# compbioproj-cdna-to-genome-map-align/gmap-2024

Hardware: AMD Instinct MI355X
Metric: aligned cDNA reads/sec (2 kb, GRCh38) at 1/2/4/8 MI355X; DP HBM GB/s vs peak (higher is better)
Workload: dtype int32

## Files before the change

### gmap-2024_amd/csrc/s2c_kernel.hip

```cpp
#include <cstdlib>

#include "dp_device.h"
#include <climits>

namespace gmapdp {

constexpr int kS2K = 8;
constexpr int kS2EqualNotSplicing = 9;
constexpr int kS2EnoughConsec = 32;
constexpr int kS2GreedyConsec = 100;
constexpr int kS2ExonDefn = 30;
constexpr int kS2MinTerminal = 8;
constexpr int kS2MaxNactive = 100;
constexpr int kS2MaxSkipped = 3;
constexpr int kS2ScoreRestrict = 10;
constexpr int kS2TenThousand = 8192;
constexpr int kS2FinalTolerance = 20;
constexpr int kS2MaxNalignments = 10;
constexpr int kS2Sufflookback = 60, kS2Nsufflookback = 5;
constexpr int kS2ExtraBounds = 20;
constexpr int kS2cCap = 4096;

#ifdef GMAPDP_OI_TIMING
__device__ unsigned long long g_s2_marks[2][16];
__device__ unsigned int g_s2_wave[3][16384];
__device__ unsigned long long g_s2_sub[2][8];
#define S2_SUB_DECL() unsigned long long _sub_t0 = 0
#define S2_SUB_T0() (_sub_t0 = wall_clock64())
#define S2_SUB(k) (W.sub[k] += wall_clock64() - _sub_t0, W.subn[k]++)
#define S2_MARK(k)                                                  \
  do {                                                              \
    if (threadIdx.x == 0) {                                         \
      atomicAdd(&g_s2_marks[0][k], (unsigned long long)wall_clock64()); \
      atomicAdd(&g_s2_marks[1][k], 1ull);                           \
    }                                                               \
  } while (0)
#define S2_COUNT(k, v)                                             \
  do {                                                              \
    if (threadIdx.x == 0) atomicAdd(&g_s2_marks[0][k], (unsigned long long)(v)); \
  } while (0)
#else
#define S2_MARK(k) \
  do {             \
  } while (0)
#define S2_COUNT(k, v) \
  do {                 \
  } while (0)
#define S2_SUB_DECL() (void)0
#define S2_SUB_T0() (void)0
#define S2_SUB(k) (void)0
#endif

constexpr int kS2NoPositions = 0, kS2Coverage = 1, kS2Chained = 2, kS2Overflow = -2, kS2Domain = -3;

struct __attribute__((aligned(16))) S2Hit {
  int consec, root, tracei, pred;
};
struct S2Diag {
  uint32_t diagonal;
  int querystart, queryend, nconsecutive, dominatedp, pad_;
  double score;
};
struct S2Path {
  int cell;
  int n;
  uint32_t start, end;
};
struct S2Scratch {
  size_t diff, run, off, minact, maxact, first, proc, diags, ord, tmp, hits, maps, sc, cand, keep, paths, pq, ph, lh,
      sbuf, total;
  int sortn;
};
__host__ __device__ inline int s2_pow2(int n) {
  int p = 64;
  while (p < n) p <<= 1;
  return p;
}
__host__ __device__ inline S2Scratch s2_scratch(int ql, int T, int nd) {
  S2Scratch s;
  const size_t Q = (size_t)ql + 1, D = (size_t)(nd > 0 ? nd : 1), H = (size_t)(T > 0 ? T : 1);
  s.diff = 0;
  s.run = align16(s.diff + 4 * Q);
  s.off = align16(s.run + 8 * Q);
  s.minact = align16(s.off + 4 * Q);
  s.maxact = align16(s.minact + 4 * Q);
  s.first = align16(s.maxact + 4 * Q);
  s.proc = align16(s.first + 4 * Q);
  s.diags = align16(s.proc + 4 * Q);
  s.ord = align16(s.diags + sizeof(S2Diag) * D);
  s.tmp = align16(s.ord + 4 * D);
  s.hits = align16(s.tmp + 4 * D);
  s.maps = align16(s.hits + sizeof(S2Hit) * H);
  s.sc = align16(s.maps + 4 * H);
  s.cand = align16(s.sc + 4 * H);
  s.keep = align16(s.cand + 4 * H);
  s.paths = align16(s.keep + 4 * H);
  s.pq = align16(s.paths + sizeof(S2Path) * H);
  s.ph = align16(s.pq + 4 * Q);
  s.lh = align16(s.ph + 4 * Q);
  s.sortn = s2_pow2((int)(H > D ? H : D));
  s.sbuf = align16(s.lh + 8 * Q);
  s.total = align16(s.sbuf + 4 * (size_t)s.sortn);
  return s;
}

__device__ __forceinline__ int wave_incl_sum(int x, int lane) {
#pragma unroll
  for (int off = 1; off < 64; off <<= 1) {
    const int y = __shfl_up(x, off, 64);
    if (lane >= off) x += y;
  }
  return x;
}
__device__ __forceinline__ int wave_incl_max(int x, int lane) {
#pragma unroll
  for (int off = 1; off < 64; off <<= 1) {
    const int y = __shfl_up(x, off, 64);
    if (lane >= off) x = max(x, y);
  }
  return x;
}
__device__ __forceinline__ int wave_max_i(int x) {
#pragma unroll
  for (int off = 32; off >= 1; off >>= 1) x = max(x, __shfl_xor(x, off, 64));
  return x;
}
__device__ __forceinline__ int wave_sum_i(int x) {
#pragma unroll
  for (int off = 32; off >= 1; off >>= 1) x += __shfl_xor(x, off, 64);
  return x;
}
__device__ __forceinline__ void wave_sync() { __syncthreads(); }

template <class Less>
__device__ void wave_sort(int lane, int n, const int* in, int* out, int* sbuf, Less less) {
  if (n <= 0) return;
  const int NN = s2_pow2(n);
  for (int i = lane; i < NN; i += 64) sbuf[i] = i < n ? i : -1;
  wave_sync();
  auto lt = [&](int x, int y) {
    if (x < 0) return false;
    if (y < 0) return true;
    const int vx = in[x], vy = in[y];
    if (less(vx, vy)) return true;
    if (less(vy, vx)) return false;
    return x < y;
  };
  for (int size = 2; size <= NN; size <<= 1) {
    for (int stride = size >> 1; stride > 0; stride >>= 1) {
      for (int i = lane; i < NN; i += 64) {
        const int j = i ^ stride;
        if (j > i) {
          const int a = sbuf[i], b = sbuf[j];
          const bool up = (i & size) == 0;
          if (up ? lt(b, a) : lt(a, b)) {
            sbuf[i] = b;
            sbuf[j] = a;
          }
        }
      }
      wave_sync();
    }
  }
  for (int i = lane; i < n; i += 64) out[i] = in[sbuf[i]];
  wave_sync();
}

template <class F>
__device__ __forceinline__ void fill_range(int lane, uint32_t* dst, int a, int b, F f) {
  for (int q = a + lane; q <= b; q += 64) dst[q] = f(q);
}

struct S2Best {
  int consec, root, pp, ph, score, tracei;
// ... 543 lines not shown
  }
  s2_uniform(b);
  bool donep = false;
  int last_tr = -1;
  if (np > 0 && b.consec < kS2EnoughConsec) {
    S2_SUB_T0();
    S2Pref pf;
    pf.load(W, np);
    const uint64_t dm = ballot(W.lane < np && W.lane > nlookback && (q - pf.q) - kS2K > lookback);
    const int kmax = dm ? __ffsll((long long)dm) - 1 : (np <= 64 ? np - 1 : 64);
    int fdummy = 0, lt = -1, from = 0;
    S2_SUB(1);
    int st;
    S2_SUB_T0();
    st = s2_dloop_fast(W, pf, np, kmax, q, position, b, W.splicingp != 0, false, fdummy, lt);
    S2_SUB(2);
    S2_SUB_T0();
    if (st == 2) from = 64;
    if (!st) {
      const int kg = kmax >= 64 ? 63 : kmax;
      S2Pref pg = pf;
      for (;;) {
        int nb = from;
        st = s2_dloop_multi(W, pg, np, kg, q, position, b, W.splicingp != 0, false, fdummy, lt, from, &nb);
        if (st != 2) break;
        from = nb;
        pg.load(W, np, from);
      }
      if (st == 1 && kmax >= 64 && b.consec < kS2EnoughConsec) {
        st = 2;
        from = 64;
      }
    }
    S2_SUB(3);
    S2_SUB_T0();
    if (st == 1) np = 0;
    if (st != 1) last_tr = lt;
    S2EntryCache ec;
    for (int kk = from; kk < np && b.consec < kS2EnoughConsec && !donep; kk++) {
      const int eq = kk < kS2Pref ? __builtin_amdgcn_readlane(pf.q, kk) : ec.get(W, np, kk).q;
      if (kk > nlookback && (q - eq) - kS2K > lookback) donep = true;
      int qd;
      (void)s2_entry_eval(W, pf, ec, np, kk, 0, q, position, last_tr, b, W.splicingp != 0, &qd);
    }
    S2_SUB(4);
  }
  s2_uniform(b);
  if (b.pp < 0) {
    b.tracei = ++W.tracectr;
    b.score = kS2K;
  }
  return b;
}

__device__ __forceinline__ void s2_store_link(S2W& W, int offq, int hit, const S2Best& b) {
  if (W.lane == 0) {
    W.hits[offq + hit] = S2Hit{b.consec, b.root, b.tracei, b.ph};
    W.sc[offq + hit] = b.score;
  }
}

__device__ __forceinline__ void s2_mult(S2W& W, int q, int offq, int low, int high, int np, const S2E& last) {
  int* fr = s2_fr;
  const int nhits = high - low;
  if (np == 0) {
    for (int i = W.lane; i < nhits; i += 64) {
      W.hits[offq + low + i] = S2Hit{kS2K, (int)W.maps[offq + low + i], W.tracectr + 1 + i, -1};
      W.sc[offq + low + i] = kS2K;
    }
    W.tracectr += nhits;
    wave_sync();
    return;
  }
  const int adq = q - last.q;
  int maxadj = 0, maxnon = 0, nfr = 0;
  S2EntryCache ec;
  for (int n = 0; n < np && n < 128; n++) {
    const S2E e = ec.get(W, np, n);
    const int qd = q - e.q;
    if (n > kS2Nsufflookback && n > 1 && qd - kS2K > kS2Sufflookback) break;
    if (n <= 1 || qd - kS2K <= kS2Sufflookback / 2) maxadj = n;
    if (n <= kS2Nsufflookback || qd - kS2K <= kS2Sufflookback) maxnon = n;
    if (W.lane == 0) fr[n] = e.n > 0 ? 0 : -1;
    nfr = n + 1;
  }
  wave_sync();
  int overall = 0, adjf = last.n > 0 ? 0 : -1;
  for (int i = 0; i < nhits; i++) {
    const uint32_t position = W.maps[offq + low + i];
    S2HV u;
    if (s2_adj(W, last, adjf, adq, position, u) && u.consec + adq > overall) overall = u.consec + adq;
  }
  adjf = last.n > 0 ? 0 : -1;
  for (int i = 0; i < nhits; i++) {
    const uint32_t position = W.maps[offq + low + i];
    S2Best b;
    int maxseen;
    S2HV u;
    if (s2_adj(W, last, adjf, adq, position, u)) {
      b = {u.consec + adq, u.root, last.q, u.hit, u.score + adq, u.tracei};
      maxseen = maxadj;
    } else {
      b = {kS2K, (int)position, -1, -1, 0, -1};
      maxseen = maxnon;
    }
    if (overall < kS2GreedyConsec) {
      int last_tr = -1;
      for (int kk = 0; kk < np && b.consec < kS2EnoughConsec && kk <= maxseen && kk < nfr; kk++) {
        const int f = s2_u(s2_fr[kk]);
        if (f != -1) {
          const S2E e = ec.get(W, np, kk);
          const int nf = s2_eval(W, e, f, q, position, last_tr, b, true);
          wave_sync();
          if (W.lane == 0) fr[kk] = nf;
          wave_sync();
        }
      }
    }
    if (b.pp < 0) {
      b.tracei = ++W.tracectr;
      b.score = kS2K;
    }
    s2_store_link(W, offq, low + i, b);
  }
  wave_sync();
}

struct S2Run {
  int score, consec, tracei, root, hit, q, pushed, np;
};
__device__ __forceinline__ void s2_run_write(S2Hit* hits, int* sc, int* alist, int lane, int off, int hit,
                                             int prev, uint32_t map, int qq, S2Run L, uint64_t Mm) {
  if (!((Mm >> lane) & 1ull)) return;
  const uint64_t below = Mm & ((1ull << lane) - 1ull);
  const int r = __popcll(below);
  const int dq = qq - L.q;
  hits[off + hit] = S2Hit{L.consec + dq, L.root, L.tracei, below ? prev : L.hit};
  sc[off + hit] = L.score + dq;
  alist[off] = hit;
  const int sl = (L.pushed + r) & (kS2Ring - 1);
  s2_ring.map[sl] = map;
  s2_ring.score[sl] = L.score + dq;
  s2_ring.consec[sl] = L.consec + dq;
  s2_ring.tracei[sl] = L.tracei;
  s2_ring.root[sl] = L.root;
  s2_ring.hit[sl] = off + hit;
  const int ms = (L.np + r) & (kS2Meta - 1);
  s2_ring.eq[ms] = qq;
  s2_ring.en[ms] = 1;
  s2_ring.eoff[ms] = off;
  s2_ring.estart[ms] = L.pushed + r;
}

__device__ __forceinline__ void s2_sweep(S2W& W, const int32_t* npq, int nq, const int* lowa, const int* higha,
                                         const uint32_t* rmapa, int qstart, int qend) {
  const int lane = W.lane;
  auto npos = [&](int q) { return q < nq ? npq[q] : 0; };
  int q = 0, np = 0;
  for (int i = lane; i < qstart; i += 64) W.actn[i] = 0;
  q = qstart;
  while (q <= qend && npos(q) <= 0) {
    if (lane == 0) W.actn[q] = 0;
    q++;
  }
  if (q <= qend) {
    const int n = npos(q), offq = W.off[q];
    for (int i = lane; i < n; i += 64) {
      W.hits[offq + i] = S2Hit{kS2K, 0, -1, -1};
      W.sc[offq + i] = kS2K;
    }
  }
  wave_sync();
  int grand_score = 0, grand_q = -1, grand_hit = -1, nskipped = 0, min_hits = 1000000, specific_q = -1,
      specific_low = 0, specific_high = 0;
  uint32_t grand_map = 0;
  S2E last = {0, 0, 0, 0, false};
  int cb = -1, m_n = 0, m_off = 0, m_low = 0, m_high = 0;
  uint32_t m_rmap = 0;
#ifdef GMAPDP_OI_TIMING
  unsigned long long t_one = 0, t_mult = 0, t_tail = 0, t_meta = 0, t0c = 0;
#define S2_T0() t0c = wall_clock64()
#define S2_TACC(acc) (acc += wall_clock64() - t0c, t0c = wall_clock64())
#else
#define S2_T0() (void)0
#define S2_TACC(acc) (void)0
#endif
  while (q <= qend) {
    S2_T0();
    W.tracectr = s2_u(W.tracectr);
    W.pushed = s2_u(W.pushed);
    if ((q & ~63) != cb) {
      cb = q & ~63;
      const int qq = cb + lane;
      const bool in = qq <= qend;
      m_n = qq < nq ? npq[qq] : 0;
      m_off = qq <= qend + 1 ? W.off[qq] : 0;
      m_low = in ? lowa[qq] : 0;
      m_high = in ? higha[qq] : 0;
      m_rmap = in ? rmapa[qq] : 0u;
    }
    const int j = q - cb;
    if (last.n == 1 && last.inring && nskipped <= kS2MaxSkipped) {
      const int ls = last.start & (kS2Ring - 1);
      const uint32_t lmap = s2_u(s2_ring.map[ls]);
      const int lcons = s2_u(s2_ring.consec[ls]);
      const uint32_t dg = lmap - (uint32_t)last.q;
      const int qq = cb + lane;
      const bool one = qq <= qend && m_high - m_low == 1 && m_rmap - (uint32_t)qq == dg;
      const uint64_t from_j = ~0ull << j;
      const uint64_t notE = ~ballot(qq <= qend && (m_n <= 0 || one)) & from_j;
      const int stop = notE ? __ffsll((long long)notE) - 1 : 64;
      const uint64_t inrun = stop >= 64 ? from_j : (from_j & ((1ull << stop) - 1ull));
      const uint64_t Mm = ballot(one) & inrun;
      if (Mm && lcons + (cb + __ffsll((long long)Mm) - 1 - last.q) >= kS2EnoughConsec) {
        const int lscore = s2_u(s2_ring.score[ls]), ltr = s2_u(s2_ring.tracei[ls]), lroot = s2_u(s2_ring.root[ls]),
                  lhit = s2_u(s2_ring.hit[ls]);
        const uint64_t mb = Mm & ((1ull << lane) - 1ull);
        const int prev = __shfl(m_off + m_low, mb ? 63 - __clzll((long long)mb) : 0, 64);
        s2_run_write(W.hits, W.sc, W.alist, lane, m_off, m_low, prev, m_rmap, qq,
                     {lscore, lcons, ltr, lroot, lhit, last.q, W.pushed, np}, Mm);
        if ((inrun >> lane) & 1ull) W.actn[qq] = (int)((Mm >> lane) & 1ull);
        const int cnt = __popcll(Mm);
        S2_TALLY(n_runs, 1);
        S2_TALLY(n_runpos, cnt);
        const int ll = 63 - __clzll((long long)Mm);
        const int lq = cb + ll;
        const int lsc = lscore + (lq - last.q);
        if (lsc >= grand_score) {
          grand_score = lsc;
          grand_q = lq;
          grand_hit = __builtin_amdgcn_readlane(m_off + m_low, ll);
          grand_map = (uint32_t)__builtin_amdgcn_readlane((int)m_rmap, ll);
        }
        const int loff = __builtin_amdgcn_readlane(m_off, ll);
        W.pushed += cnt;
        np += cnt;
        last = s2_mkentry(W, lq, 1, loff, W.pushed - 1);
        nskipped = 0;
        min_hits = 1000000;
        specific_q = -1;
        __atomic_signal_fence(__ATOMIC_SEQ_CST);
        __builtin_amdgcn_wave_barrier();
        S2_TACC(t_one);
        q = cb + stop;
        continue;
      }
    }
    const int n = __builtin_amdgcn_readlane(m_n, j);
    const int offq = __builtin_amdgcn_readlane(m_off, j);
    int low = __builtin_amdgcn_readlane(m_low, j), high = __builtin_amdgcn_readlane(m_high, j);
    if (high - low >= kS2MaxNactive && nskipped <= kS2MaxSkipped) {
      if (lane == 0) W.actn[q] = 0;
      nskipped++;
      if (high - low < min_hits) {
        min_hits = high - low;
        specific_q = q;
        specific_low = low;
        specific_high = high;
      }
      q++;
      continue;
    }
    int next_q, qoff = offq;
    if (nskipped > kS2MaxSkipped) {
      next_q = q;
      q = specific_q;
      low = specific_low;
      high = specific_high;
      qoff = W.off[q];
    } else {
      next_q = q + 1;
    }
    S2_TACC(t_meta);
    int nact = 0;
    if (high - low == 1) {
      const uint32_t position = (q == cb + j) ? (uint32_t)__builtin_amdgcn_readlane((int)m_rmap, j)
                                              : W.maps[qoff + low];
      S2Best b = s2_one(W, q, position, np, last);
      int best_score = b.score > 0 ? b.score : 0;
      const bool have_best = b.score > 0;
      nskipped = 0;
      min_hits = 1000000;
      specific_q = -1;
      if (W.splicingp && have_best && b.ph < 0 && grand_q >= 0 && q >= grand_q + kS2K) {
        if ((best_score = grand_score - (q - grand_q)) > 0) {
          if (!(position > grand_map + W.maxintronlen) && position >= grand_map + (uint32_t)kS2K) {
            b.consec = kS2K;
            b.pp = grand_q;
            b.ph = grand_hit;
            b.tracei = ++W.tracectr;
            b.score = best_score;
          }
        }
      }
      if (have_best && best_score >= grand_score && b.consec > kS2ExonDefn) {
        grand_score = best_score;
        grand_q = q;
        grand_hit = qoff + low;
        grand_map = position;
      }
      s2_store_link(W, qoff, low, b);
      const int threshold = max(b.score - kS2ScoreRestrict, 0);
      if (b.score > threshold) {
        nact = 1;
        if (lane == 0) {
          W.alist[qoff] = low;
          const int sl = W.pushed & (kS2Ring - 1);
          s2_ring.map[sl] = position;
          s2_ring.score[sl] = b.score;
          s2_ring.consec[sl] = b.consec;
          s2_ring.tracei[sl] = b.tracei;
          s2_ring.root[sl] = b.root;
          s2_ring.hit[sl] = qoff + low;
        }
      }
    } else if (high - low > 1 && high - low <= 64) {
      const int nh = high - low;
      S2_SUB_DECL();
      S2_SUB_T0();
      const uint32_t cm = lane < nh ? W.maps[qoff + low + lane] : 0u;
      S2Best mb = {0, 0, -1, -1, 0, 0};
      if (np == 0) {
        if (lane < nh) mb = {kS2K, (int)cm, -1, -1, kS2K, W.tracectr + 1 + lane};
        W.tracectr += nh;
      } else {
        const int adq = q - last.q;
        S2Pref pf;
        pf.load(W, np);
        S2EntryCache ec;
        int maxadj = 0, maxnon = 0, nfr = 0;
        for (int base = 0; base < np && base < 128; base += 64) {
          const int n = base + lane;
          const bool in = n < np && n < 128;
          int eq = pf.q, en = pf.n;
          if (base) {
            const int k = (np - 1 - n) & (kS2Meta - 1);
            eq = in ? s2_ring.eq[k] : 0;
            en = in ? s2_ring.en[k] : 0;
          }
          const int qd = q - eq;
          const uint64_t B = ballot(in && n > kS2Nsufflookback && n > 1 && qd - kS2K > kS2Sufflookback);
          const int lim = B ? __ffsll((long long)B) - 1 : 64;
          const bool v = in && lane < lim;
          const uint64_t A = ballot(v && (n <= 1 || qd - kS2K <= kS2Sufflookback / 2));
          const uint64_t M = ballot(v && (n <= kS2Nsufflookback || qd - kS2K <= kS2Sufflookback));
          if (A) maxadj = base + 63 - __clzll((long long)A);
          if (M) maxnon = base + 63 - __clzll((long long)M);
          if (v) s2_fr[n] = en > 0 ? 0 : -1;
          const uint64_t Vm = ballot(v);
          if (Vm) nfr = base + 64 - __clzll((long long)Vm);
          if (B || !(Vm >> 63)) break;
// ... 534 lines not shown
          t.y = __builtin_amdgcn_readlane(vi.y, j);
          acc += *reinterpret_cast<const double*>(&t);
          if (lane == j) pre = acc;
        }
        if (q < ql) run[q] = pre;
      }
    }
    wave_sync();
    for (int d = lane; d < nd; d += 64) dg[d].score = run[dg[d].queryend] - run[dg[d].querystart];
    wave_sync();
    int ngood = 0;
    for (int cb = 0; cb < nd; cb += 64) {
      const int d = nd - 1 - (cb + lane);
      const bool g = (cb + lane < nd) && dg[d].score >= 10.0;
      const uint64_t m = ballot(g);
      if (g) ord[ngood + lanes_below(m, lane)] = d;
      ngood += __popcll(m);
    }
    if (ngood == 0) {
      for (int d = lane; d < nd; d += 64) ord[d] = d;
      ngood = nd;
    }
    wave_sync();
    wave_sort(lane, ngood, ord, tmp, sbuf, [&](int a, int b) { return dg[a].nconsecutive > dg[b].nconsecutive; });
    int nunique = ngood;
    for (int i = 0; i < nunique; i++) {
      const S2Diag sup = dg[tmp[i]];
      const int expected = sup.queryend + 1 - sup.querystart;
      int threshold;
      if (expected < 100 && sup.nconsecutive > expected - 10) {
        threshold = sup.nconsecutive - 20;
      } else if (expected >= 100 && sup.nconsecutive > expected * 0.90) {
        threshold = (int)(sup.nconsecutive * 0.80);
      } else {
        continue;
      }
      int k = i + 1;
      for (int cb = i + 1; cb < nunique; cb += 64) {
        const int j = cb + lane;
        int d = -1;
        bool live = false;
        if (j < nunique) {
          d = tmp[j];
          S2Diag& sub = dg[d];
          if (sub.querystart >= sup.querystart && sub.queryend <= sup.queryend && sub.nconsecutive < threshold)
            sub.dominatedp = 1;
          live = !sub.dominatedp;
        }
        const uint64_t m = ballot(live);
        wave_sync();
        if (live) tmp[k + lanes_below(m, lane)] = d;
        k += __popcll(m);
        wave_sync();
      }
      nunique = k;
    }
    wave_sort(lane, nunique, tmp, ord, sbuf, [&](int a, int b) { return dg[a].diagonal < dg[b].diagonal; });
    if (nunique > 100) {
      if (lane == 0) {
        const uint32_t mind = dg[ord[0]].diagonal, maxd = dg[ord[nunique - 1]].diagonal;
        const int nbins = (int)((maxd - mind) / 10000) + 1;
        int maxcount = 0, curbin = -1, curcount = 0;
        uint32_t center = 0;
        for (int i = 0; i <= nunique; i++) {
          const int b = i < nunique ? (int)((dg[ord[i]].diagonal - mind) / 10000) : nbins;
          if (b != curbin) {
            if (curbin >= 0 && curcount > maxcount) {
              maxcount = curcount;
              center = mind + 10000u * (uint32_t)curbin;
            }
            curbin = b;
            curcount = 0;
          }
          curcount++;
        }
        center += 5000;
        int j = 0;
        for (int i = 0; i < nunique; i++) {
          const uint32_t dd = dg[ord[i]].diagonal;
          if (!(dd + 10000 < center || dd > center + 10000)) ord[j++] = ord[i];
        }
        sh[0] = j;
      }
      wave_sync();
      nunique = sh[0];
    }
    const S2Diag d0 = dg[ord[0]], dl = dg[ord[nunique - 1]];
    qstart = ql - 1;
    qend = 0;
    {
      int mn = ql - 1, mx = 0;
      for (int i = lane; i < nunique; i += 64) {
        mn = min(mn, dg[ord[i]].querystart);
        mx = max(mx, dg[ord[i]].queryend);
      }
      qstart = -wave_max_i(-mn);
      qend = wave_max_i(mx);
    }
    auto minline = [&](uint32_t diagonal) {
      return [=](int q) {
        return (diagonal + (uint32_t)q < (uint32_t)kS2ExtraBounds) ? chrinit
                                                                    : chrinit + diagonal + (uint32_t)q - kS2ExtraBounds;
      };
    };
    auto maxline = [&](uint32_t diagonal) {
      return [=](int q) {
        const uint32_t position = diagonal + (uint32_t)q + kS2ExtraBounds;
        return (position > genomiclength) ? chrterm : chrinit + position;
      };
    };
    fill_range(lane, minact, 0, d0.querystart - 1, [&](int) { return 0u; });
    int q = d0.querystart;
    uint32_t diagonal = d0.diagonal;
    fill_range(lane, minact, q, d0.queryend, minline(diagonal));
    q = max(q, d0.queryend + 1);
    for (int i = 0, j; i < nunique; i = j) {
      const int qe_i = dg[ord[i]].queryend;
      for (j = i + 1; j < nunique && dg[ord[j]].queryend <= qe_i; j++) ;
      if (j < nunique) {
        diagonal = dg[ord[i]].diagonal;
        const int b = dg[ord[j]].queryend;
        fill_range(lane, minact, q, b, minline(diagonal));
        q = max(q, b + 1);
      }
    }
    {
      const uint32_t dlast = diagonal;
      fill_range(lane, minact, q, ql - 1, [=](int qq) {
        return (dlast + (uint32_t)qq < (uint32_t)kS2ExtraBounds) ? chrinit : chrinit + (uint32_t)qq - kS2ExtraBounds;
      });
    }
    const int activeend = dl.queryend;
    fill_range(lane, maxact, activeend + 1, ql - 1, [&](int) { return chrterm; });
    q = min(ql - 1, activeend);
    diagonal = dl.diagonal;
    fill_range(lane, maxact, dl.querystart, q, maxline(diagonal));
    q = min(q, dl.querystart - 1);
    for (int i = nunique - 1, j; i >= 0; i = j) {
      const int qs_i = dg[ord[i]].querystart;
      for (j = i - 1; j >= 0 && dg[ord[j]].querystart > qs_i; j--) ;
      if (j >= 0) {
        diagonal = dg[ord[i]].diagonal;
        const int a = dg[ord[j]].querystart;
        fill_range(lane, maxact, a, q, maxline(diagonal));
        q = min(q, a - 1);
      }
    }
    fill_range(lane, maxact, 0, q, maxline(diagonal));
  }
  R.diag_querystart = qstart;
  R.diag_queryend = qend;

  S2_MARK(2);
  int* lowa = reinterpret_cast<int*>(S + so.lh);
  int* higha = lowa + (ql + 1);
  uint32_t* mapsa = reinterpret_cast<uint32_t*>(S + so.maps);
  int* sca = reinterpret_cast<int*>(S + so.sc);
  const bool records = T <= kS2cCap && nq <= 65536;
  uint32_t* rmapa = reinterpret_cast<uint32_t*>(diff);
  carry = 0;
  bool big = false;
  uint32_t pmap = 0;
  for (int cb = 0; cb < ql; cb += 64) {
    const int q = cb + lane;
    const int v = q < nq ? npq[q] : 0;
    const int incl = carry + wave_incl_sum(v, lane);
    const int o = incl - v;
    if (q < ql) off[q] = o;
    const int mq = q < nq && v > 0 ? mpq[q] : 0;
    const bool act = q <= qend && v > 0;
    const uint32_t qmn = act ? minact[q] : 0u, qmx0 = act ? maxact[q] : 0u;
    const uint32_t qmx = (qmn > 0 && qmx0 < qmn - 1) ? qmn - 1 : qmx0;
    if (q < ql && !act) {
      lowa[q] = higha[q] = 0;
      rmapa[q] = 0u;
    }
    const int hend = __shfl(incl, 63, 64);
    for (int base = carry; base < hend; base += 64) {
      const int h = base + lane;
      int j = 0;
#pragma unroll
      for (int st = 32; st >= 1; st >>= 1) {
        const int oj = __shfl(o, j + st, 64);
        if (oj <= h) j += st;
      }
      const int oq = __shfl(o, j, 64), mj = __shfl(mq, j, 64), nj = __shfl(v, j, 64);
      const uint32_t mn = (uint32_t)__shfl((int)qmn, j, 64), mx = (uint32_t)__shfl((int)qmx, j, 64);
      const bool actj = __shfl(act ? 1 : 0, j, 64) != 0;
      uint32_t map = 0u;
      if (h < hend) {
        map = table_all[O.table_offset + mj + (h - oq)];
        big |= (map >= 0x80000000u);
        if (records) hits[h] = S2Hit{0, 0, 0, 0};
        mapsa[h] = map;
        sca[h] = 0;
      }
      uint32_t prev = (uint32_t)__shfl_up((int)map, 1, 64);
      if (lane == 0) prev = pmap;
      if (h < hend && actj) {
        const int k = h - oq, qj = cb + j;
        const bool first = k == 0, last = k == nj - 1;
        if (map >= mn && (first || prev < mn)) {
          lowa[qj] = k;
          rmapa[qj] = map <= mx ? map : 0u;
        } else if (last && map < mn) {
          lowa[qj] = nj;
          rmapa[qj] = 0u;
        }
        if (map > mx && (first || prev <= mx)) higha[qj] = k;
        else if (last && map <= mx) higha[qj] = nj;
      }
      pmap = (uint32_t)__builtin_amdgcn_readlane((int)map, 63);
    }
    carry = hend;
  }
  if (lane == 0) off[ql] = carry;
  if (ballot(big)) {
    if (lane == 0) {
      R.status = kS2Domain;
      results[P.index] = R;
    }
    return;
  }
  wave_sync();
  {
    int wk = 0;
    for (int q = qstart + lane; q <= qend; q += 64) {
      const int d = higha[q] - lowa[q];
      wk += d > 0 ? 1 + 4 * (d - 1) : 0;
    }
    wk = wave_sum_i(wk);
    if (lane == 0) work[pos] = wk;
  }

  if (lane == 0) results[P.index] = R;
}

#ifndef GMAPDP_S2B_WPE
#define GMAPDP_S2B_WPE 4
#endif
__global__ __launch_bounds__(64) __attribute__((amdgpu_waves_per_eu(GMAPDP_S2B_WPE))) void s2b_kernel(
    const DevStage2Problem* __restrict__ probs, const uint32_t* __restrict__ blocks, uint64_t nwords,
    const char* __restrict__ qseq, const char* __restrict__ quc, const gmapdp_oligo_result* __restrict__ ores,
    const int32_t* __restrict__ npos_all, const int32_t* __restrict__ map_all, const uint32_t* __restrict__ table_all,
    const int32_t* __restrict__ diag_all, unsigned char* __restrict__ scratch, unsigned long long* __restrict__ counters,
    unsigned long long scratch_cap, gmapdp_stage2_result* __restrict__ results, gmapdp_path* __restrict__ paths_out,
    unsigned long long path_cap, gmapdp_path_pair* __restrict__ pairs_out, unsigned long long pair_cap) {
  __shared__ int sh[8];
  const int lane = threadIdx.x;
  const DevStage2Problem P = probs[s2_problem(counters)];
  const int ql = P.querylength, nq = ql - kS2K + 1;
  const gmapdp_oligo_result O = ores[P.index];
  const int T = O.totalpositions, nd = O.ndiagonals;
  const int32_t* npq = npos_all + P.qoff;
  const int32_t* mpq = map_all + P.qoff;
  const S2Scratch so = s2_scratch(ql, T, nd);
  unsigned char* S = scratch + P.scratch_offset;
  int* diff = reinterpret_cast<int*>(S + so.diff);
  double* run = reinterpret_cast<double*>(S + so.run);
  int* off = reinterpret_cast<int*>(S + so.off);
  uint32_t* minact = reinterpret_cast<uint32_t*>(S + so.minact);
  uint32_t* maxact = reinterpret_cast<uint32_t*>(S + so.maxact);
  int* first = reinterpret_cast<int*>(S + so.first);
  int* proc = reinterpret_cast<int*>(S + so.proc);
  S2Diag* dg = reinterpret_cast<S2Diag*>(S + so.diags);
  int* ord = reinterpret_cast<int*>(S + so.ord);
  int* tmp = reinterpret_cast<int*>(S + so.tmp);
  S2Hit* hits = reinterpret_cast<S2Hit*>(S + so.hits);
  int* cand = reinterpret_cast<int*>(S + so.cand);
  int* keep = reinterpret_cast<int*>(S + so.keep);
  S2Path* pth = reinterpret_cast<S2Path*>(S + so.paths);
  int* pathq = reinterpret_cast<int*>(S + so.pq);
  int* pathh = reinterpret_cast<int*>(S + so.ph);
  int* sbuf = reinterpret_cast<int*>(S + so.sbuf);
  (void)sh; (void)diff; (void)run; (void)off; (void)minact; (void)maxact; (void)first; (void)proc; (void)dg;
  (void)ord; (void)tmp; (void)hits; (void)cand; (void)keep; (void)pth; (void)pathq; (void)pathh; (void)sbuf;
  (void)npq; (void)mpq; (void)nq; (void)blocks; (void)nwords; (void)qseq; (void)quc; (void)table_all;
  (void)diag_all; (void)counters; (void)scratch_cap; (void)paths_out; (void)path_cap; (void)pairs_out; (void)pair_cap;
  const gmapdp_stage2_result R0 = results[P.index];
  if (R0.status != kS2Chained) return;
  const int qstart = R0.diag_querystart, qend = R0.diag_queryend;
  S2_MARK(3);
#ifdef GMAPDP_OI_TIMING
  const unsigned long long tw0 = wall_clock64();
#endif
  {
    S2W W;
    W.hits = hits;
    W.maps = reinterpret_cast<const uint32_t*>(S + so.maps);
    W.sc = reinterpret_cast<int*>(S + so.sc);
    W.off = off;
    W.actn = first;
    W.alist = keep;
    W.pq = proc;
    W.pn = pathq;
    W.poff = pathh;
    W.pstart = reinterpret_cast<int*>(run);
    W.pushed = 0;
    W.tracectr = 0;
    W.splicingp = P.splicingp;
    W.lane = lane;
    W.maxintronlen = P.maxintronlen;
    const int* lowa = reinterpret_cast<const int*>(S + so.lh);
    s2_sweep(W, npq, nq, lowa, lowa + (ql + 1), reinterpret_cast<const uint32_t*>(diff), qstart,
             qend);
  }
  wave_sync();
#ifdef GMAPDP_OI_TIMING
  if (lane == 0 && P.index < 16384) {
    g_s2_wave[0][P.index] = (unsigned int)(wall_clock64() - tw0);
    g_s2_wave[1][P.index] = (unsigned int)(qend - qstart + 1);
    g_s2_wave[2][P.index] = (unsigned int)T;
  }
#endif

  S2_MARK(4);
}

constexpr uint32_t kS2NoPred = 0x7fffu;
struct S2WalkOut {
  int n, top, bottom;
};
__device__ S2WalkOut s2_walk_diag(const S2Hit* __restrict__ hits, const uint32_t* __restrict__ maps,
                                  const int* __restrict__ scs, const int* __restrict__ off, int ql, int gi, int lane,
                                  int* __restrict__ pq, int* __restrict__ ph) {
  S2WalkOut o = {0, -1, -1};
  while (gi >= 0 && hits[gi].consec < kS2MinTerminal) gi = hits[gi].pred;
  int qn = -1;
  while (gi >= 0) {
    if (qn < 0) qn = s2_hit_pos_wave(off, ql, gi, lane);
    int p = qn - lane;
    int lo = p >= 0 ? off[p] : 0, hi = p >= 0 ? off[p + 1] : 0;
    if (!(s2_u(lo) <= gi && gi < s2_u(hi))) {
      qn = s2_hit_pos_wave(off, ql, gi, lane);
      p = qn - lane;
      lo = p >= 0 ? off[p] : 0;
      hi = p >= 0 ? off[p + 1] : 0;
    }
    const uint32_t mn = s2_u(maps[gi]);
    const uint32_t target = mn - (uint32_t)lane;
    int idx = -1;
    if (lane == 0) {
      idx = gi;
    } else if (p >= 0) {
      const int end = hi;
      while (lo < hi) {
        const int mid = (lo + hi) >> 1;
        if (maps[mid] < target) lo = mid + 1;
        else hi = mid;
      }
      if (lo < end && maps[lo] == target) idx = lo;
    }
    int sc = 0;
    S2Hit x = {0, 0, 0, -1};
    if (idx >= 0) {
      sc = scs[idx];
      x = hits[idx];
    }
    if (lane > 0 && sc <= 0) idx = -1;
    const int pred = idx >= 0 ? x.pred : -1;
    const uint32_t mx = idx >= 0 ? target : 0x80000000u;
    const int qx = p;
    const int prev_pred = __shfl_up(pred, 1, 64);
    const bool c = lane == 0 || (idx >= 0 && prev_pred == idx);
    const uint64_t brk = ballot(!c);
    const int len = brk ? __ffsll((long long)brk) - 1 : 64;
    const bool vis = lane < len && (int)mx >= 0;
    const uint64_t vm = ballot(vis);
    if (vis && pq) {
      const int k = o.n + lanes_below(vm, lane);
      pq[k] = qx;
      ph[k] = (int)mx;
    }
    if (vm) {
      const int f = __ffsll((long long)vm) - 1, l = 63 - __clzll((long long)vm);
      if (o.top < 0) o.top = __builtin_amdgcn_readlane(idx, f);
      o.bottom = __builtin_amdgcn_readlane(idx, l);
    }
    o.n += __popcll(vm);
    gi = __builtin_amdgcn_readlane(pred, len - 1);
    qn = max(qn - len, -1);
  }
  return o;
}

__device__ S2WalkOut s2_walk_wave(const uint32_t* lql, const uint32_t* map, int gi, int lane, int* pq, int* ph) {
  S2WalkOut o = {0, -1, -1};
  uint32_t w = lql[gi];
  while (w & 0x8000u) {
    const uint32_t pr = w & kS2NoPred;
    if (pr == kS2NoPred) return o;
    gi = (int)pr;
    w = lql[gi];
  }
  for (;;) {
    const int x = gi - lane;
    const uint32_t wx = x >= 0 ? lql[x] : kS2NoPred;
    const uint32_t px = wx & kS2NoPred;
    const bool cont = x >= 1 && px == (uint32_t)(x - 1);
    const uint64_t stop = ballot(!cont);
    const int r = stop ? __ffsll((long long)stop) - 1 : 63;
    const uint32_t mx = lane <= r ? map[x] : 0x80000000u;
    const bool vis = (int)mx >= 0;
    const uint64_t vm = ballot(vis);
    if (vis && pq) {
      const int idx = o.n + lanes_below(vm, lane);
      pq[idx] = (int)(wx >> 16);
      ph[idx] = (int)mx;
    }
    if (vm) {
      if (o.top < 0) o.top = gi - (__ffsll((long long)vm) - 1);
      o.bottom = gi - (63 - __clzll((long long)vm));
    }
    o.n += __popcll(vm);
    const uint32_t pr = (uint32_t)__builtin_amdgcn_readlane((int)px, r);
    if (pr == kS2NoPred) return o;
    gi = (int)pr;
  }
}

template <bool kLdsWalk>
__global__ __launch_bounds__(64) void s2c_kernel(
    const DevStage2Problem* __restrict__ probs, const uint32_t* __restrict__ blocks, uint64_t nwords,
    const char* __restrict__ qseq, const char* __restrict__ quc, const gmapdp_oligo_result* __restrict__ ores,
    const int32_t* __restrict__ npos_all, const int32_t* __restrict__ map_all, const uint32_t* __restrict__ table_all,
    const int32_t* __restrict__ diag_all, unsigned char* __restrict__ scratch, unsigned long long* __restrict__ counters,
    unsigned long long scratch_cap, gmapdp_stage2_result* __restrict__ results, gmapdp_path* __restrict__ paths_out,
    unsigned long long path_cap, gmapdp_path_pair* __restrict__ pairs_out, unsigned long long pair_cap) {
  __shared__ int sh[8];
  const int lane = threadIdx.x;
  const DevStage2Problem P = probs[s2_problem(counters)];
  const int ql = P.querylength, nq = ql - kS2K + 1;
  const gmapdp_oligo_result O = ores[P.index];
  const int T = O.totalpositions, nd = O.ndiagonals;
  const int32_t* npq = npos_all + P.qoff;
  const int32_t* mpq = map_all + P.qoff;
  const S2Scratch so = s2_scratch(ql, T, nd);
  unsigned char* S = scratch + P.scratch_offset;
  int* diff = reinterpret_cast<int*>(S + so.diff);
  double* run = reinterpret_cast<double*>(S + so.run);
  int* off = reinterpret_cast<int*>(S + so.off);
  uint32_t* minact = reinterpret_cast<uint32_t*>(S + so.minact);
  uint32_t* maxact = reinterpret_cast<uint32_t*>(S + so.maxact);
  int* first = reinterpret_cast<int*>(S + so.first);
  int* proc = reinterpret_cast<int*>(S + so.proc);
  S2Diag* dg = reinterpret_cast<S2Diag*>(S + so.diags);
  int* ord = reinterpret_cast<int*>(S + so.ord);
  int* tmp = reinterpret_cast<int*>(S + so.tmp);
  S2Hit* hits = reinterpret_cast<S2Hit*>(S + so.hits);
  const uint32_t* maps = reinterpret_cast<const uint32_t*>(S + so.maps);
  const int* scs = reinterpret_cast<const int*>(S + so.sc);
  int* cand = reinterpret_cast<int*>(S + so.cand);
  int* keep = reinterpret_cast<int*>(S + so.keep);
  S2Path* pth = reinterpret_cast<S2Path*>(S + so.paths);
  int* pathq = reinterpret_cast<int*>(S + so.pq);
  int* pathh = reinterpret_cast<int*>(S + so.ph);
  int* sbuf = reinterpret_cast<int*>(S + so.sbuf);
  (void)sh; (void)diff; (void)run; (void)off; (void)minact; (void)maxact; (void)first; (void)proc; (void)dg;
  (void)ord; (void)tmp; (void)hits; (void)cand; (void)keep; (void)pth; (void)pathq; (void)pathh; (void)sbuf;
  (void)npq; (void)mpq; (void)nq; (void)blocks; (void)nwords; (void)qseq; (void)quc; (void)table_all;
  (void)diag_all; (void)counters; (void)scratch_cap; (void)paths_out; (void)path_cap; (void)pairs_out; (void)pair_cap;
  gmapdp_stage2_result R = results[P.index];
  if (R.status != kS2Chained) return;
  if ((T <= kS2cCap && nq <= 65536) != kLdsWalk) return;
  S2_MARK(12);
  const int qstart = R.diag_querystart, qend = R.diag_queryend;
  const int h0 = off[qstart], h1 = off[qend + 1];
  const int H = T > 0 ? T : 1;
  int* cq = reinterpret_cast<int*>(pth);
  int* croot = cq + H;
  int* slots = croot + H;
  int* sorted = slots + H;
  int best = 0, ncand = 0;
  {
    const int* __restrict__ scr = scs;
    int* __restrict__ cw = cand;
    int* __restrict__ kw = keep;
    constexpr int kB = 8;
    for (int cb = h0; cb < h1; cb += 64 * kB) {
      int sc[kB];
#pragma unroll
      for (int k = 0; k < kB; k++) {
        const int gi = cb + 64 * k + lane;
        sc[k] = gi < h1 ? scr[gi] : 0;
      }
#pragma unroll
      for (int k = 0; k < kB; k++) {
        const int gi = cb + 64 * k + lane;
        best = max(best, wave_max_i(sc[k]));
        const bool c = gi < h1 && sc[k] > best - kS2FinalTolerance && sc[k] > 0;
        const uint64_t m = ballot(c);
        if (c) {
          cw[ncand + lanes_below(m, lane)] = gi;
          kw[ncand + lanes_below(m, lane)] = sc[k];
        }
        ncand += __popcll(m);
      }
    }
  }
  wave_sync();
  if (best > 0) {
    int n2 = 0;
    for (int cb = 0; cb < ncand; cb += 64) {
      const int i = cb + lane;
      const int gi = i < ncand ? cand[i] : 0, sc = i < ncand ? keep[i] : 0;
      const bool c = i < ncand && sc > best - kS2FinalTolerance;
      const uint64_t m = ballot(c);
      if (c) {
        const int s = n2 + lanes_below(m, lane);
        cand[s] = gi;
        keep[s] = sc;
        cq[s] = s2_hit_pos(off, ql, gi);
        croot[s] = hits[gi].root;
        slots[s] = s;
      }
      n2 += __popcll(m);
    }
    ncand = n2;
  } else {
    ncand = 0;
  }
  wave_sync();
  wave_sort(lane, ncand, slots, sorted, sbuf, [&](int a, int b) {
    if (croot[a] != croot[b]) return croot[a] < croot[b];
    if (keep[a] != keep[b]) return keep[a] > keep[b];
    if (cq[a] != cq[b]) return cq[a] > cq[b];
    return cand[a] < cand[b];
  });
  int nkeep = 0, gcarry = 0;
  for (int cb = 0; cb < ncand; cb += 64) {
    const int i = cb + lane;
    int s = 0, gstart = 0;
    if (i < ncand) {
      s = sorted[i];
      gstart = (i == 0 || croot[sorted[i - 1]] != croot[s]) ? i : 0;
    }
    int m = gstart;
#pragma unroll
    for (int o = 1; o < 64; o <<= 1) {
      const int y = __shfl_up(m, o, 64);
      if (lane >= o) m = max(m, y);
    }
    m = max(m, gcarry);
    gcarry = __shfl(m, 63, 64);
    const bool k = i < ncand && keep[s] == keep[sorted[m]];
    const uint64_t bm = ballot(k);
    if (k) slots[nkeep + lanes_below(bm, lane)] = s;
    nkeep += __popcll(bm);
  }
  wave_sync();
  wave_sort(lane, nkeep, slots, sorted, sbuf, [&](int a, int b) {
    if (keep[a] != keep[b]) return keep[a] > keep[b];
    if (croot[a] != croot[b]) return croot[a] < croot[b];
    if (cq[a] != cq[b]) return cq[a] > cq[b];
    return cand[a] < cand[b];
  });
  for (int i = lane; i < nkeep; i += 64) slots[i] = cand[sorted[i]];
  wave_sync();
  for (int i = lane; i < nkeep; i += 64) cand[i] = slots[i];
  wave_sync();
  int npaths = 0;
  while (npaths < nkeep && (npaths < kS2MaxNalignments || scs[cand[npaths]] == best)) npaths++;
  R.npaths = npaths;

  S2_MARK(5);
  extern __shared__ uint32_t s2c_lds[];
  uint32_t* llq = s2c_lds;
  uint32_t* lmap = s2c_lds + kS2cCap;
  const bool lds_walk = kLdsWalk;
  if (lds_walk && npaths > 0) {
    const S2Hit* __restrict__ hr = hits;
    const uint32_t* __restrict__ mr = maps;
    const int* __restrict__ offr = off;
    for (int cb = 0; cb < ql; cb += 64) {
      const int o = offr[min(cb + lane, ql)];
      const int hbeg = __shfl(o, 0, 64), hend = s2_u(offr[min(cb + 64, ql)]);
      for (int base = hbeg; base < hend; base += 64) {
        const int h = base + lane;
        int j = 0;
#pragma unroll
        for (int st = 32; st >= 1; st >>= 1) {
          const int oj = __shfl(o, j + st, 64);
          if (oj <= h) j += st;
        }
        if (h < hend) {
          const S2Hit x = hr[h];
          const uint32_t pr = x.pred >= 0 ? (uint32_t)x.pred : kS2NoPred;
          llq[h] = ((uint32_t)(cb + j) << 16) | (x.consec < kS2MinTerminal ? 0x8000u : 0u) | pr;
          lmap[h] = mr[h];
        }
      }
    }
  }
  wave_sync();
#ifdef GMAPDP_OI_TIMING
  if (threadIdx.x == 0) {
    atomicAdd(&g_s2_marks[1][13], (unsigned long long)npaths);
    atomicAdd(&g_s2_marks[1][14], (unsigned long long)wall_clock64());
  }
#endif
  const bool single = npaths == 1;
  for (int p = 0; p < npaths; p++) {
    const int cell = s2_u(cand[p]);
    int n = 0, top = -1, bottom = -1;
    if (lds_walk || nq <= 65536) {
      const S2WalkOut o = lds_walk ? s2_walk_wave(llq, lmap, cell, lane, single ? pathq : nullptr, pathh)
                                   : s2_walk_diag(hits, maps, scs, off, ql, cell, lane, single ? pathq : nullptr, pathh);
      n = o.n;
      top = o.top;
      bottom = o.bottom;
    } else if (lane == 0) {
      s2_walk(hits, maps, off, ql, cell, [&](int gi, int q) {
        if (n == 0) top = gi;
        bottom = gi;
        if (single) {
          pathq[n] = q;
          pathh[n] = (int)maps[gi];
// ... 262 lines not shown
```

Measured before the change: 340,400.

## Lay out only in-window hits per query, using per-query binary search for bounds

The hit layout pass now finds each query position's low/high window bounds by a short linear scan or binary search over its sorted table slice. It then writes only the hits inside that window, except at the first active query, which keeps all its hits. Previously every seeded hit was copied and bounds were derived by comparing neighbours. This cuts the scratch writes and the downstream sweep's hit count, and folds the work estimate into the same pass. In exchange, offsets and the sweep's low/high semantics change, and the domain-overflow check becomes a conservative range test plus a last-element check.

```diff
diff --git a/gmap-2024_amd/csrc/s2c_kernel.hip b/gmap-2024_amd/csrc/s2c_kernel.hip
--- a/gmap-2024_amd/csrc/s2c_kernel.hip
+++ b/gmap-2024_amd/csrc/s2c_kernel.hip
@@ -20,6 +20,12 @@
 constexpr int kS2Sufflookback = 60, kS2Nsufflookback = 5;
 constexpr int kS2ExtraBounds = 20;
 constexpr int kS2cCap = 4096;
+#ifndef GMAPDP_S2C_CLASS_LAID
+#define GMAPDP_S2C_CLASS_LAID 0
+#endif
+__host__ __device__ inline bool s2c_lds_class(int seeded, int laid, int nq) {
+  return (GMAPDP_S2C_CLASS_LAID ? laid : seeded) <= kS2cCap && nq <= 65536;
+}
 
 #ifdef GMAPDP_OI_TIMING
 __device__ unsigned long long g_s2_marks[2][16];
@@ -869,8 +875,8 @@
   s2_ring.estart[ms] = L.pushed + r;
 }
 
-__device__ __forceinline__ void s2_sweep(S2W& W, const int32_t* npq, int nq, const int* lowa, const int* higha,
-                                         const uint32_t* rmapa, int qstart, int qend) {
+__device__ __forceinline__ void s2_sweep(S2W& W, const int32_t* npq, int nq, const int* fp, const uint32_t* rmapa,
+                                         int qstart, int qend) {
   const int lane = W.lane;
   auto npos = [&](int q) { return q < nq ? npq[q] : 0; };
   int q = 0, np = 0;
@@ -880,8 +886,12 @@
     if (lane == 0) W.actn[q] = 0;
     q++;
   }
+  const int q0 = q;
+  int low0 = 0, high0 = 0;
   if (q <= qend) {
     const int n = npos(q), offq = W.off[q];
+    low0 = s2_u(fp[0]);
+    high0 = s2_u(fp[1]);
     for (int i = lane; i < n; i += 64) {
       W.hits[offq + i] = S2Hit{kS2K, 0, -1, -1};
       W.sc[offq + i] = kS2K;
@@ -912,8 +922,9 @@
       const bool in = qq <= qend;
       m_n = qq < nq ? npq[qq] : 0;
       m_off = qq <= qend + 1 ? W.off[qq] : 0;
-      m_low = in ? lowa[qq] : 0;
-      m_high = in ? higha[qq] : 0;
+      const int o1 = in ? W.off[qq + 1] : 0;
+      m_low = qq == q0 ? low0 : 0;
+      m_high = qq == q0 ? high0 : o1 - m_off;
       m_rmap = in ? rmapa[qq] : 0u;
     }
     const int j = q - cb;
@@ -1754,28 +1765,77 @@
   R.diag_queryend = qend;
 
   S2_MARK(2);
-  int* lowa = reinterpret_cast<int*>(S + so.lh);
-  int* higha = lowa + (ql + 1);
+  int* fp = reinterpret_cast<int*>(S + so.lh);
   uint32_t* mapsa = reinterpret_cast<uint32_t*>(S + so.maps);
   int* sca = reinterpret_cast<int*>(S + so.sc);
-  const bool records = T <= kS2cCap && nq <= 65536;
   uint32_t* rmapa = reinterpret_cast<uint32_t*>(diff);
+  const uint32_t* __restrict__ tb = table_all + O.table_offset;
+  wave_sync();
+  int q0 = -1;
+  for (int cb = qstart & ~63; cb <= qend && q0 < 0; cb += 64) {
+    const int q = cb + lane;
+    const uint64_t m = ballot(q >= qstart && q <= qend && q < nq && npq[q] > 0);
+    if (m) q0 = cb + __ffsll((long long)m) - 1;
+  }
+  const bool scan_big = (uint64_t)chrinit + (uint64_t)genomiclength + (uint64_t)ql + 64u >= 0x80000000ull;
   carry = 0;
   bool big = false;
-  uint32_t pmap = 0;
+  int wk = 0;
   for (int cb = 0; cb < ql; cb += 64) {
     const int q = cb + lane;
     const int v = q < nq ? npq[q] : 0;
-    const int incl = carry + wave_incl_sum(v, lane);
-    const int o = incl - v;
-    if (q < ql) off[q] = o;
-    const int mq = q < nq && v > 0 ? mpq[q] : 0;
+    const int mq = v > 0 ? mpq[q] : 0;
     const bool act = q <= qend && v > 0;
     const uint32_t qmn = act ? minact[q] : 0u, qmx0 = act ? maxact[q] : 0u;
     const uint32_t qmx = (qmn > 0 && qmx0 < qmn - 1) ? qmn - 1 : qmx0;
-    if (q < ql && !act) {
-      lowa[q] = higha[q] = 0;
-      rmapa[q] = 0u;
+    if (scan_big && v > 0) big |= (tb[mq + v - 1] >= 0x80000000u);
+    int low = 0, high = 0;
+    uint32_t rmap = 0u;
+    if (act) {
+      const uint32_t* __restrict__ sl = tb + mq;
+      if (v <= 4) {
+        uint32_t e[4];
+#pragma unroll
+        for (int k = 0; k < 4; k++) e[k] = k < v ? sl[k] : 0u;
+#pragma unroll
+        for (int k = 0; k < 4; k++) {
+          low += (k < v && e[k] < qmn) ? 1 : 0;
+          high += (k < v && e[k] <= qmx) ? 1 : 0;
+        }
+        high = max(high, low);
+        const uint32_t el = low == 0 ? e[0] : low == 1 ? e[1] : low == 2 ? e[2] : e[3];
+        rmap = high > low ? el : 0u;
+      } else {
+        int lo = 0, hi = v;
+        while (lo < hi) {
+          const int mid = (lo + hi) >> 1;
+          if (sl[mid] < qmn) lo = mid + 1;
+          else hi = mid;
+        }
+        low = lo;
+        hi = v;
+        while (lo < hi) {
+          const int mid = (lo + hi) >> 1;
+          if (sl[mid] <= qmx) lo = mid + 1;
+          else hi = mid;
+        }
+        high = lo;
+        rmap = high > low ? sl[low] : 0u;
+      }
+    }
+    if (q >= qstart && q <= qend && high > low) wk += 1 + 4 * (high - low - 1);
+    int c = high - low, first_hit = mq + low;
+    if (q == q0) {
+      fp[0] = low;
+      fp[1] = high;
+      c = v;
+      first_hit = mq;
+    }
+    const int incl = carry + wave_incl_sum(c, lane);
+    const int o = incl - c;
+    if (q < ql) {
+      off[q] = o;
+      rmapa[q] = rmap;
     }
     const int hend = __shfl(incl, 63, 64);
     for (int base = carry; base < hend; base += 64) {
@@ -1786,37 +1846,17 @@
         const int oj = __shfl(o, j + st, 64);
         if (oj <= h) j += st;
       }
-      const int oq = __shfl(o, j, 64), mj = __shfl(mq, j, 64), nj = __shfl(v, j, 64);
-      const uint32_t mn = (uint32_t)__shfl((int)qmn, j, 64), mx = (uint32_t)__shfl((int)qmx, j, 64);
-      const bool actj = __shfl(act ? 1 : 0, j, 64) != 0;
-      uint32_t map = 0u;
+      const int oq = __shfl(o, j, 64), fj = __shfl(first_hit, j, 64);
       if (h < hend) {
-        map = table_all[O.table_offset + mj + (h - oq)];
-        big |= (map >= 0x80000000u);
-        if (records) hits[h] = S2Hit{0, 0, 0, 0};
-        mapsa[h] = map;
+        mapsa[h] = tb[fj + (h - oq)];
         sca[h] = 0;
       }
-      uint32_t prev = (uint32_t)__shfl_up((int)map, 1, 64);
-      if (lane == 0) prev = pmap;
-      if (h < hend && actj) {
-        const int k = h - oq, qj = cb + j;
-        const bool first = k == 0, last = k == nj - 1;
-        if (map >= mn && (first || prev < mn)) {
-          lowa[qj] = k;
-          rmapa[qj] = map <= mx ? map : 0u;
-        } else if (last && map < mn) {
-          lowa[qj] = nj;
-          rmapa[qj] = 0u;
-        }
-        if (map > mx && (first || prev <= mx)) higha[qj] = k;
-        else if (last && map <= mx) higha[qj] = nj;
-      }
-      pmap = (uint32_t)__builtin_amdgcn_readlane((int)map, 63);
     }
     carry = hend;
   }
   if (lane == 0) off[ql] = carry;
+  if (s2c_lds_class(T, carry, nq))
+    for (int h = lane; h < carry; h += 64) hits[h] = S2Hit{0, 0, 0, 0};
   if (ballot(big)) {
     if (lane == 0) {
       R.status = kS2Domain;
@@ -1825,15 +1865,8 @@
     return;
   }
   wave_sync();
-  {
-    int wk = 0;
-    for (int q = qstart + lane; q <= qend; q += 64) {
-      const int d = higha[q] - lowa[q];
-      wk += d > 0 ? 1 + 4 * (d - 1) : 0;
-    }
-    wk = wave_sum_i(wk);
-    if (lane == 0) work[pos] = wk;
-  }
+  wk = wave_sum_i(wk);
+  if (lane == 0) work[pos] = wk;
 
   if (lane == 0) results[P.index] = R;
 }
@@ -1903,8 +1936,7 @@
     W.splicingp = P.splicingp;
     W.lane = lane;
     W.maxintronlen = P.maxintronlen;
-    const int* lowa = reinterpret_cast<const int*>(S + so.lh);
-    s2_sweep(W, npq, nq, lowa, lowa + (ql + 1), reinterpret_cast<const uint32_t*>(diff), qstart,
+    s2_sweep(W, npq, nq, reinterpret_cast<const int*>(S + so.lh), reinterpret_cast<const uint32_t*>(diff), qstart,
              qend);
   }
   wave_sync();
@@ -2064,7 +2096,7 @@
   (void)diag_all; (void)counters; (void)scratch_cap; (void)paths_out; (void)path_cap; (void)pairs_out; (void)pair_cap;
   gmapdp_stage2_result R = results[P.index];
   if (R.status != kS2Chained) return;
-  if ((T <= kS2cCap && nq <= 65536) != kLdsWalk) return;
+  if (s2c_lds_class(T, off[ql], nq) != kLdsWalk) return;
   S2_MARK(12);
   const int qstart = R.diag_querystart, qend = R.diag_queryend;
   const int h0 = off[qstart], h1 = off[qend + 1];
```

Measured after the change: 346,900 (median of 6 runs). 1.02x the previous value.
